# francescofugazzi/3dgsconverter

Hardware: NVIDIA H100
Metric: Msplats/s SOR k=16 (higher is better)
Workload: dtype f32

## Files before the change

3dgsconverter_b200/csrc/gsx_radix.cu:

```cuda
#include "../../include/gsx.h"

#include "gsx_common.cuh"
#include "gsx_radix.cuh"

namespace gsx {

#define GSX_FULL 0xffffffffu
constexpr int kRsThreads = 256;
constexpr int kRsPerThread = 16;
constexpr int kRsTile = kRsThreads * kRsPerThread;
constexpr int kRsWarpKeys = 32 * kRsPerThread;
constexpr int kScanBlock = 2048;

__global__ void __launch_bounds__(256) k_scan_block(uint32_t* __restrict__ data, int64_t n,
                                                    uint32_t* __restrict__ sums) {
    const int64_t base = (int64_t)blockIdx.x * kScanBlock + (int64_t)threadIdx.x * 8;
    uint32_t v[8];
    uint32_t tsum = 0;
#pragma unroll
    for (int e = 0; e < 8; ++e) {
        v[e] = base + e < n ? data[base + e] : 0u;
        tsum += v[e];
    }
    uint32_t x = tsum;
// ... 114 lines not shown
    __syncthreads();
    uint32_t dcount;
    {
        const int d = threadIdx.x;
        uint32_t run = 0;
#pragma unroll
        for (int ww = 0; ww < 8; ++ww) {
            uint32_t c = wcnt[ww][d];
            wcnt[ww][d] = run;
            run += c;
        }
        dcount = run;
        gbase[d] = base_off[(size_t)d * ntiles + blockIdx.x];
    }
    {
        uint32_t x = dcount;
#pragma unroll
        for (int o = 1; o < 32; o <<= 1) {
            uint32_t y = __shfl_up_sync(GSX_FULL, x, o);
            if (lane >= o) x += y;
        }
        __shared__ uint32_t wtot[8];
        if (lane == 31) wtot[w] = x;
        __syncthreads();
        uint32_t woff = 0;
#pragma unroll
        for (int i = 0; i < 8; ++i)
            if (i < w) woff += wtot[i];
        dstart[threadIdx.x] = woff + x - dcount;
    }
    __syncthreads();
#pragma unroll
    for (int e = 0; e < kRsPerThread; ++e) {
        const int64_t i = wbase + e * 32 + lane;
        if (i < n) {
            const uint32_t d = (uint32_t)(key[e] >> shift) & dmask;
            const uint32_t lp = dstart[d] + wcnt[w][d] + rank[e];
            skeys[lp] = key[e];
            svals[lp] = vals_in[i];
        }
    }
    __syncthreads();
    const int cnt = (int)(n - tbase < kRsTile ? n - tbase : kRsTile);
    for (int j = threadIdx.x; j < cnt; j += kRsThreads) {
        const uint64_t k = skeys[j];
        const uint32_t d = (uint32_t)(k >> shift) & dmask;
        const uint32_t pos = gbase[d] + ((uint32_t)j - dstart[d]);
        keys_out[pos] = k;
        vals_out[pos] = svals[j];
    }
}

constexpr uint32_t kOsAgg = 1u << 30, kOsInc = 1u << 31, kOsVal = (1u << 30) - 1u;
constexpr int kOsMaxPass = 8;
constexpr uint32_t kOsSpinLimit = 1u << 22;

__global__ void __launch_bounds__(256) k_os_hist(const uint64_t* __restrict__ keys, int64_t n, int begin_bit,
                                                  int npass, uint32_t last_mask, uint32_t* __restrict__ ghist) {
    __shared__ uint32_t sh[kOsMaxPass * 256];
    for (int t = threadIdx.x; t < npass * 256; t += 256) sh[t] = 0;
    __syncthreads();
    const int64_t stride = (int64_t)gridDim.x * 256;
    for (int64_t i = (int64_t)blockIdx.x * 256 + threadIdx.x; i < n; i += stride) {
        const uint64_t k = keys[i] >> begin_bit;
        for (int p = 0; p < npass; ++p)
            atomicAdd(&sh[p * 256 + ((uint32_t)(k >> (8 * p)) & (p == npass - 1 ? last_mask : 255u))], 1u);
    }
    __syncthreads();
    for (int t = threadIdx.x; t < npass * 256; t += 256)
        if (sh[t]) atomicAdd(&ghist[t], sh[t]);
}

__global__ void __launch_bounds__(256) k_os_scan(uint32_t* __restrict__ ghist) {
    uint32_t* h = ghist + blockIdx.x * 256;
    const int lane = threadIdx.x & 31, w = threadIdx.x >> 5;
    const uint32_t v = h[threadIdx.x];
    uint32_t x = v;
#pragma unroll
    for (int o = 1; o < 32; o <<= 1) {
        uint32_t y = __shfl_up_sync(GSX_FULL, x, o);
        if (lane >= o) x += y;
    }
    __shared__ uint32_t wt[8];
    if (lane == 31) wt[w] = x;
    __syncthreads();
    uint32_t woff = 0;
#pragma unroll
    for (int i = 0; i < 8; ++i)
        if (i < w) woff += wt[i];
    h[threadIdx.x] = woff + x - v;
}

template <bool PAIRS>
constexpr size_t os_pass_smem() {
    return (size_t)kRsTile * (PAIRS ? 12 : 8) + (size_t)8 * 256 * 4 + 2 * 256 * 4;
}

template <bool PAIRS>
__global__ void __launch_bounds__(kRsThreads, PAIRS ? 3 : 4)
    k_os_pass(const uint64_t* __restrict__ keys_in, const int32_t* __restrict__ vals_in, uint64_t* __restrict__ keys_out,
              int32_t* __restrict__ vals_out, int64_t n, int shift, uint32_t dmask, const uint32_t* __restrict__ gbase_pass,
              uint32_t* lookback, unsigned int* tile_counter) {
    extern __shared__ __align__(16) unsigned char rs_smem[];
    uint64_t* skeys = reinterpret_cast<uint64_t*>(rs_smem);
    int32_t* svals = reinterpret_cast<int32_t*>(rs_smem + (size_t)kRsTile * 8);
    constexpr size_t kPairBytes = (size_t)kRsTile * (PAIRS ? 12 : 8);
    uint32_t(*wcnt)[256] = reinterpret_cast<uint32_t(*)[256]>(rs_smem + kPairBytes);
    uint32_t* dstart = reinterpret_cast<uint32_t*>(rs_smem + kPairBytes + 8 * 256 * 4);
    uint32_t* gbase = dstart + 256;
    __shared__ unsigned int s_tile;
    const int lane = threadIdx.x & 31, w = threadIdx.x >> 5;
    if (threadIdx.x == 0) s_tile = atomicAdd(tile_counter, 1u);
    for (int t = threadIdx.x; t < 8 * 256; t += kRsThreads) (&wcnt[0][0])[t] = 0;
    __syncthreads();
    const unsigned int tile = s_tile;
    const int64_t tbase = (int64_t)tile * kRsTile;
    const int64_t wbase = tbase + (int64_t)w * kRsWarpKeys;
    uint64_t key[kRsPerThread];
    uint32_t rank2[kRsPerThread / 2];
#pragma unroll
    for (int e = 0; e < kRsPerThread; ++e) {
        const int64_t i = wbase + e * 32 + lane;
        key[e] = i < n ? keys_in[i] : 0ull;
// ... 30 lines not shown
        for (int64_t t = (int64_t)tile - 1; t >= 0; --t) {
            uint32_t v, spins = 0;
            while (((v = lb[(size_t)t * 256 + d]) & (kOsAgg | kOsInc)) == 0u)
                if (++spins > kOsSpinLimit) __trap();
            excl += v & kOsVal;
            if (v & kOsInc) break;
        }
        if (tile != 0) lb[(size_t)tile * 256 + d] = (excl + dcount) | kOsInc;
        gbase[d] = gbase_pass[d] + excl;
    }
    {
        uint32_t x = dcount;
#pragma unroll
        for (int o = 1; o < 32; o <<= 1) {
            uint32_t y = __shfl_up_sync(GSX_FULL, x, o);
            if (lane >= o) x += y;
        }
        __shared__ uint32_t wtot[8];
        if (lane == 31) wtot[w] = x;
        __syncthreads();
        uint32_t woff = 0;
#pragma unroll
        for (int i = 0; i < 8; ++i)
            if (i < w) woff += wtot[i];
        dstart[threadIdx.x] = woff + x - dcount;
    }
    __syncthreads();
#pragma unroll
    for (int e = 0; e < kRsPerThread; ++e) {
        const int64_t i = wbase + e * 32 + lane;
        if (i < n) {
            const uint32_t d = (uint32_t)(key[e] >> shift) & dmask;
            const uint32_t lp = dstart[d] + wcnt[w][d] + ((rank2[e >> 1] >> (16 * (e & 1))) & 0xffffu);
            skeys[lp] = key[e];
            if (PAIRS) svals[lp] = vals_in[i];
        }
    }
    __syncthreads();
    const int cnt = (int)(n - tbase < kRsTile ? n - tbase : kRsTile);
    for (int j = threadIdx.x; j < cnt; j += kRsThreads) {
        const uint64_t k = skeys[j];
        const uint32_t d = (uint32_t)(k >> shift) & dmask;
        const uint32_t pos = gbase[d] + ((uint32_t)j - dstart[d]);
        keys_out[pos] = k;
        if (PAIRS) vals_out[pos] = svals[j];
    }
}

static size_t os_ws_elems(int64_t n) {
    const int64_t ntiles = (n + kRsTile - 1) / kRsTile;
    return (size_t)kOsMaxPass * 256 + 64 + (size_t)kOsMaxPass * 256 * ntiles;
}

template <bool PAIRS>
static int onesweep_sort(uint64_t* keys0, uint64_t* keys1, int32_t* vals0, int32_t* vals1, int64_t n, int begin_bit,
                         int end_bit, uint32_t* ws, uint64_t** keys_sorted, int32_t** vals_sorted, cudaStream_t st) {
    const int64_t ntiles = (n + kRsTile - 1) / kRsTile;
    const int npass = (end_bit - begin_bit + 7) / 8;
    uint32_t* ghist = ws;
    unsigned int* counters = ws + kOsMaxPass * 256;
    uint32_t* lookback = ws + kOsMaxPass * 256 + 64;
    GSX_CUDA_CHECK(cudaMemsetAsync(ws, 0, ((size_t)kOsMaxPass * 256 + 64 + (size_t)npass * 256 * ntiles) * sizeof(uint32_t), st));
    static int hist_blocks = 0;
    if (!hist_blocks) {
        int dev = 0, sms = 132;
        cudaGetDevice(&dev);
        cudaDeviceGetAttribute(&sms, cudaDevAttrMultiProcessorCount, dev);
        hist_blocks = sms * 8;
    }
    int64_t hb = (n + 255) / 256;
    if (hb > hist_blocks) hb = hist_blocks;
    const uint32_t last_mask = digit_mask(begin_bit + 8 * (npass - 1), end_bit);
    k_os_hist<<<(unsigned)hb, 256, 0, st>>>(keys0, n, begin_bit, npass, last_mask, ghist);
    GSX_KERNEL_CHECK();
    k_os_scan<<<npass, 256, 0, st>>>(ghist);
    GSX_KERNEL_CHECK();
    GSX_CUDA_CHECK(cudaFuncSetAttribute(k_os_pass<PAIRS>, cudaFuncAttributeMaxDynamicSharedMemorySize, (int)os_pass_smem<PAIRS>()));
    uint64_t *kin = keys0, *kout = keys1;
    int32_t *vin = vals0, *vout = vals1;
    for (int p = 0; p < npass; ++p) {
        k_os_pass<PAIRS><<<(unsigned)ntiles, kRsThreads, os_pass_smem<PAIRS>(), st>>>(
            kin, vin, kout, vout, n, begin_bit + 8 * p, p == npass - 1 ? last_mask : 255u, ghist + p * 256,
            lookback + (size_t)p * 256 * ntiles, counters + p);
        GSX_KERNEL_CHECK();
        uint64_t* tk = kin;
        kin = kout;
        kout = tk;
        int32_t* tv = vin;
        vin = vout;
        vout = tv;
    }
    *keys_sorted = kin;
    if (vals_sorted) *vals_sorted = vin;
    return GSX_OK;
}

size_t radix_ws_bytes(int64_t n) {
    if (n < 1) n = 1;
    int64_t ntiles = (n + kRsTile - 1) / kRsTile;
    size_t hist = (size_t)256 * ntiles;
    size_t three_kernel = hist + scan_ws_elems((int64_t)hist) + 256;
    size_t onesweep = os_ws_elems(n);
    return (three_kernel > onesweep ? three_kernel : onesweep) * sizeof(uint32_t);
}

int radix_sort_pairs(uint64_t* keys0, uint64_t* keys1, int32_t* vals0, int32_t* vals1, int64_t n, int begin_bit,
                     int end_bit, void* ws, size_t ws_bytes, uint64_t** keys_sorted, int32_t** vals_sorted,
                     cudaStream_t st) {
    GSX_NVTX("gsx::radix_sort_pairs");
    GSX_REQUIRE(n >= 1 && n < 4294967296ll, GSX_ERR_ARG, "radix: n out of range");
    GSX_REQUIRE(ws_bytes >= radix_ws_bytes(n), GSX_ERR_WORKSPACE, "radix: workspace too small");
    GSX_REQUIRE(begin_bit >= 0 && end_bit <= 64 && begin_bit < end_bit, GSX_ERR_ARG, "radix: bad bit range");
    if (n < (1ll << 30))
        return onesweep_sort<true>(keys0, keys1, vals0, vals1, n, begin_bit, end_bit, (uint32_t*)ws, keys_sorted,
                                   vals_sorted, st);
    const int64_t ntiles = (n + kRsTile - 1) / kRsTile;
    uint32_t* hist = (uint32_t*)ws;
    uint32_t* scan_ws = hist + (size_t)256 * ntiles;
    GSX_CUDA_CHECK(cudaFuncSetAttribute(k_rs_scatter, cudaFuncAttributeMaxDynamicSharedMemorySize, (int)kRsScatterSmem));
    uint64_t *kin = keys0, *kout = keys1;
    int32_t *vin = vals0, *vout = vals1;
    for (int shift = begin_bit; shift < end_bit; shift += 8) {
        const uint32_t dmask = digit_mask(shift, end_bit);
        k_rs_hist<<<(unsigned)ntiles, kRsThreads, 0, st>>>(kin, n, shift, dmask, ntiles, hist);
        GSX_KERNEL_CHECK();
        int rc = exclusive_scan_u32(hist, (int64_t)256 * ntiles, scan_ws, st);
        if (rc) return rc;
        k_rs_scatter<<<(unsigned)ntiles, kRsThreads, kRsScatterSmem, st>>>(kin, vin, kout, vout, n, shift, dmask, ntiles,
                                                                          hist);
        GSX_KERNEL_CHECK();
        uint64_t* tk = kin;
        kin = kout;
        kout = tk;
        int32_t* tv = vin;
        vin = vout;
        vout = tv;
    }
    *keys_sorted = kin;
    *vals_sorted = vin;
    return GSX_OK;
}

int radix_sort_keys(uint64_t* keys0, uint64_t* keys1, int64_t n, int begin_bit, int end_bit, void* ws, size_t ws_bytes,
                    uint64_t** keys_sorted, cudaStream_t st) {
    GSX_NVTX("gsx::radix_sort_keys");
    GSX_REQUIRE(n >= 1 && n < (1ll << 30), GSX_ERR_ARG, "radix: n out of range");
    GSX_REQUIRE(ws_bytes >= radix_ws_bytes(n), GSX_ERR_WORKSPACE, "radix: workspace too small");
    GSX_REQUIRE(begin_bit >= 0 && end_bit <= 64 && begin_bit < end_bit, GSX_ERR_ARG, "radix: bad bit range");
    return onesweep_sort<false>(keys0, keys1, nullptr, nullptr, n, begin_bit, end_bit, (uint32_t*)ws, keys_sorted, nullptr,
                                st);
}

}

using namespace gsx;

extern "C" {

int64_t gsx_sort_pairs_workspace_bytes(int64_t n) {
    if (n < 1) n = 1;
    return (int64_t)(align_up((size_t)n * 8, 256) + align_up((size_t)n * 4, 256) + radix_ws_bytes(n) + 1024);
}

int gsx_sort_pairs(uint64_t* keys_dev, int32_t* vals_dev, int64_t n, int32_t begin_bit, int32_t end_bit, void* ws,
                   int64_t ws_bytes, void* stream) {
    cudaStream_t st = (cudaStream_t)stream;
    if (n == 0) return GSX_OK;
    GSX_REQUIRE(ws_bytes >= gsx_sort_pairs_workspace_bytes(n), GSX_ERR_WORKSPACE, "sort: workspace too small");
    Carver c(ws, (size_t)ws_bytes);
    uint64_t* k1 = c.take<uint64_t>((size_t)n);
    int32_t* v1 = c.take<int32_t>((size_t)n);
    char* rws = c.take<char>(radix_ws_bytes(n));
    uint64_t* ks = nullptr;
    int32_t* vs = nullptr;
    int rc = vals_dev ? radix_sort_pairs(keys_dev, k1, vals_dev, v1, n, begin_bit, end_bit, rws, radix_ws_bytes(n), &ks,
                                         &vs, st)
                      : radix_sort_keys(keys_dev, k1, n, begin_bit, end_bit, rws, radix_ws_bytes(n), &ks, st);
    if (rc) return rc;
    if (ks != keys_dev) {
        GSX_CUDA_CHECK(cudaMemcpyAsync(keys_dev, ks, (size_t)n * 8, cudaMemcpyDeviceToDevice, st));
        if (vals_dev) GSX_CUDA_CHECK(cudaMemcpyAsync(vals_dev, vs, (size_t)n * 4, cudaMemcpyDeviceToDevice, st));
    }
    return GSX_OK;
}

}
```

3dgsconverter_b200/csrc/gsx_radix.cuh:

```cuda
#pragma once
#include "gsx_common.cuh"
namespace gsx {
size_t radix_ws_bytes(int64_t n);
size_t scan_workspace_bytes(int64_t n);
int exclusive_scan_u32_ws(uint32_t* data, int64_t n, uint32_t* ws, cudaStream_t st);
int radix_sort_pairs(uint64_t* keys0, uint64_t* keys1, int32_t* vals0, int32_t* vals1, int64_t n, int begin_bit,
                     int end_bit, void* ws, size_t ws_bytes, uint64_t** keys_sorted, int32_t** vals_sorted,
                     cudaStream_t st);
int radix_sort_keys(uint64_t* keys0, uint64_t* keys1, int64_t n, int begin_bit, int end_bit, void* ws, size_t ws_bytes,
                    uint64_t** keys_sorted, cudaStream_t st);
}
```

3dgsconverter_b200/csrc/gsx_sor.cu:

```cuda
#include "../../include/gsx.h"

#include "gsx_common.cuh"
#include "gsx_sor.cuh"

#include "gsx_radix.cuh"
#include <math.h>

namespace gsx {

#define GSX_D2LIM_BITS 0x60ad78ebu
#define GSX_FULL 0xffffffffu

constexpr int kCellCodeBits = 15;
constexpr float kCellCodeScale = (float)(1 << (kCellCodeBits / 3));
constexpr float kCellCodeMax = kCellCodeScale - 1.f;
constexpr int kSmallBucket = 64;
constexpr int kQueryBatch = 16;
constexpr int kMergeThreshold = 9;
constexpr int kKnnMinBlocks = 8;
constexpr int kFlatSupers = 8;
const char* sor_build_info() {
    return "knn=r03a;epi_smem=1;first_sort=1;query_batch=16;minblocks=8;merge_threshold=9;small_bucket=64;"
           "flat_supers=8;knn16=0;tma=0;i32=1;cell_order=hilbert15";
}
// ... 140 lines not shown
    }
    y ^= x, z ^= y;
    uint32_t t = 0;
#pragma unroll
    for (uint32_t q = 16; q > 1; q >>= 1)
        if (z & q) t ^= q - 1;
    x ^= t, y ^= t, z ^= t;
    return (spread6(x) << 2) | (spread6(y) << 1) | spread6(z);
}

__device__ __forceinline__ uint64_t bucket_key(float x, float y, float z, float bx, float by, float bz, float cell,
                                               int64_t n, uint64_t M64) {
    float fx, fy, fz, flx, fly, flz;
    const uint32_t h = bucket_hash(x, y, z, bx, by, bz, cell, n, M64, fx, fy, fz, flx, fly, flz);
    uint32_t sx = (uint32_t)fminf(kCellCodeMax, fmaxf(0.f, (fx - flx) * kCellCodeScale));
    uint32_t sy = (uint32_t)fminf(kCellCodeMax, fmaxf(0.f, (fy - fly) * kCellCodeScale));
    uint32_t sz = (uint32_t)fminf(kCellCodeMax, fmaxf(0.f, (fz - flz) * kCellCodeScale));
    return ((uint64_t)h << kCellCodeBits) | (uint64_t)hilbert15(sx, sy, sz);
}

struct PackFmt {
    int idx_bits, mort_bits, bucket_bits;
    __host__ __device__ int key_shift() const { return idx_bits + mort_bits; }
    __host__ __device__ uint64_t idx_mask() const { return (1ull << idx_bits) - 1ull; }
    __host__ __device__ int sort_begin() const { return idx_bits; }
    __host__ __device__ int sort_end() const { return idx_bits + mort_bits + bucket_bits; }
};

static int bits_for(int64_t n) {
    int b = 1;
    while (((int64_t)1 << b) < n) ++b;
    return b;
}

static PackFmt pack_fmt(int64_t n_items, int64_t n_buckets) {
    PackFmt f;
    f.idx_bits = bits_for(n_items);
    f.bucket_bits = bits_for(n_buckets);
    int avail = 64 - f.idx_bits - f.bucket_bits;
    if (avail > kCellCodeBits) avail = kCellCodeBits;
    f.mort_bits = avail < 0 ? 0 : avail - avail % 3;
    return f;
}

__device__ __forceinline__ uint64_t pack_word(uint64_t key , uint64_t bucket_sub,
                                              int64_t idx, PackFmt f) {
    const uint64_t bucket = (key >> kCellCodeBits) - bucket_sub;
    const uint64_t mort = (key & ((1ull << kCellCodeBits) - 1ull)) >> (kCellCodeBits - f.mort_bits);
    return (((bucket << f.mort_bits) | mort) << f.idx_bits) | (uint64_t)idx;
}

__global__ void __launch_bounds__(256) k_sor_keys(const float* __restrict__ xyz, int64_t n, float bx, float by,
                                                  float bz, float cell, uint64_t M64, PackFmt f,
                                                  uint64_t* __restrict__ keys) {
    int64_t i = (int64_t)blockIdx.x * blockDim.x + threadIdx.x;
    if (i >= n) return;
    keys[i] = pack_word(bucket_key(xyz[3 * i], xyz[3 * i + 1], xyz[3 * i + 2], bx, by, bz, cell, n, M64), 0, i, f);
}

__device__ __forceinline__ uint32_t float_to_ord(float f) {
    const uint32_t u = __float_as_uint(f);
    return (u & 0x80000000u) ? ~u : (u | 0x80000000u);
}
__device__ __forceinline__ float ord_to_float(uint32_t o) {
    return __uint_as_float((o & 0x80000000u) ? (o & 0x7fffffffu) : ~o);
}

template <bool GATHER>
__device__ __forceinline__ void
    sor_finish_tile(const int64_t tile, const float* __restrict__ xyz, const uint64_t* __restrict__ keys, PackFmt fmt,
                    float4* __restrict__ spos, int64_t n, float bx, float by, float bz, float cell, uint64_t M64,
                    int2* __restrict__ tab_se, uint32_t* __restrict__ startbits, uint32_t* __restrict__ cellbits,
                    float4* __restrict__ caabb, float4* __restrict__ saabb) {
    const int64_t j = tile * 1024 + threadIdx.x;
    const int lane = lane_id();
    float lo[3] = {INFINITY, INFINITY, INFINITY}, hi[3] = {-INFINITY, -INFINITY, -INFINITY};
    uint32_t h = 0xffffffffu;
    auto hash_at = [&](int64_t t) -> uint32_t {
        if (GATHER) return (uint32_t)(keys[t] >> fmt.key_shift());
        const float4 q = spos[t];
        return bucket_of(q.x, q.y, q.z, bx, by, bz, cell, n, M64);
    };
    int gcx = 0x7fffffff, gcy = 0, gcz = 0;
    if (j < n) {
        float x, y, z;
        if (GATHER) {
            const uint64_t word = keys[j];
            const int32_t idx = (int32_t)(word & fmt.idx_mask());
            x = xyz[3 * (int64_t)idx], y = xyz[3 * (int64_t)idx + 1], z = xyz[3 * (int64_t)idx + 2];
            spos[j] = make_float4(x, y, z, __int_as_float(idx));
            h = (uint32_t)(word >> fmt.key_shift());
        } else {
            const float4 p = spos[j];
            x = p.x, y = p.y, z = p.z;
            h = bucket_of(x, y, z, bx, by, bz, cell, n, M64);
        }
        gcx = (int)floorf(__fdiv_rn(__fsub_rn(x, bx), cell));
        gcy = (int)floorf(__fdiv_rn(__fsub_rn(y, by), cell));
        gcz = (int)floorf(__fdiv_rn(__fsub_rn(z, bz), cell));
        lo[0] = hi[0] = x;
        lo[1] = hi[1] = y;
        lo[2] = hi[2] = z;
    }
    __shared__ uint32_t sh_h[1024];
    sh_h[threadIdx.x] = h;
    __syncthreads();
    uint32_t hprev = threadIdx.x > 0 ? sh_h[threadIdx.x - 1] : 0xffffffffu;
    uint32_t hnext = threadIdx.x < 1023 ? sh_h[threadIdx.x + 1] : 0xffffffffu;
    if (j < n) {
        if (threadIdx.x == 0 && j > 0) hprev = hash_at(j - 1);
// ... 50 lines not shown
}

template <bool GATHER>
__global__ void __launch_bounds__(1024)
    k_sor_finish(const float* __restrict__ xyz, const uint64_t* __restrict__ keys, PackFmt fmt,
                 float4* __restrict__ spos, int64_t n, float bx, float by, float bz, float cell, uint64_t M64,
                 int2* __restrict__ tab_se, uint32_t* __restrict__ startbits, uint32_t* __restrict__ cellbits,
                 float4* __restrict__ caabb, float4* __restrict__ saabb) {
    sor_finish_tile<GATHER>(blockIdx.x, xyz, keys, fmt, spos, n, bx, by, bz, cell, M64, tab_se, startbits, cellbits, caabb,
                            saabb);
}

__global__ void __launch_bounds__(1024)
    k_sor_finish_gated(float4* __restrict__ spos, int64_t n, float bx, float by, float bz, float cell, uint64_t M64,
                       int2* __restrict__ tab_se, uint32_t* __restrict__ startbits, uint32_t* __restrict__ cellbits,
                       float4* __restrict__ caabb, float4* __restrict__ saabb, const unsigned int* __restrict__ gate) {
    if (!*gate) return;
    const int64_t tiles = (n + 1023) / 1024;
    for (int64_t t = blockIdx.x; t < tiles; t += gridDim.x) {
        sor_finish_tile<false>(t, nullptr, nullptr, PackFmt{}, spos, n, bx, by, bz, cell, M64, tab_se, startbits, cellbits,
                               caabb, saabb);
        __syncthreads();
    }
}

__device__ __forceinline__ void bucket_box_partial(const float4* __restrict__ spos, const float4* __restrict__ caabb,
                                                   int64_t s, int64_t end, int lane, float (&lo)[3], float (&hi)[3]) {
    lo[0] = lo[1] = lo[2] = INFINITY;
    hi[0] = hi[1] = hi[2] = -INFINITY;
    int64_t cf = (s + 31) >> 5, cl = end >> 5;
    int64_t head_end = cf * 32, tail_begin = cl * 32;
    if (cf > cl) {
        head_end = end;
        tail_begin = end;
        cf = cl = 0;
    }
    for (int64_t t = s + lane; t < head_end; t += 32) {
        float4 p = spos[t];
        lo[0] = fminf(lo[0], p.x), lo[1] = fminf(lo[1], p.y), lo[2] = fminf(lo[2], p.z);
        hi[0] = fmaxf(hi[0], p.x), hi[1] = fmaxf(hi[1], p.y), hi[2] = fmaxf(hi[2], p.z);
    }
    for (int64_t c = cf + lane; c < cl; c += 32) {
        float4 a = caabb[2 * c], b = caabb[2 * c + 1];
        lo[0] = fminf(lo[0], a.x), lo[1] = fminf(lo[1], a.y), lo[2] = fminf(lo[2], a.z);
        hi[0] = fmaxf(hi[0], a.w), hi[1] = fmaxf(hi[1], b.x), hi[2] = fmaxf(hi[2], b.y);
    }
    for (int64_t t = tail_begin + lane; t < end; t += 32) {
        float4 p = spos[t];
        lo[0] = fminf(lo[0], p.x), lo[1] = fminf(lo[1], p.y), lo[2] = fminf(lo[2], p.z);
        hi[0] = fmaxf(hi[0], p.x), hi[1] = fmaxf(hi[1], p.y), hi[2] = fmaxf(hi[2], p.z);
    }
}

__device__ __forceinline__ void
    bucket_boxes_chunk(const int64_t chunk, const uint32_t* __restrict__ startbits, const float4* __restrict__ spos,
                       const float4* __restrict__ caabb, const int2* __restrict__ tab_se, int64_t n, float bx,
                       float by, float bz, float cell, uint64_t M64, float4* __restrict__ tab_box) {
    const int lane = lane_id();
    if (chunk * 32 >= n) return;
    unsigned m = startbits[chunk];
    uint32_t my_h = 0;
    int my_end = 0;
    if ((m >> lane) & 1u) {
        const float4 p0 = spos[chunk * 32 + lane];
        my_h = bucket_of(p0.x, p0.y, p0.z, bx, by, bz, cell, n, M64);
        my_end = tab_se[my_h].y;
    }
    while (m) {
        const int src = __ffs(m) - 1;
        m &= m - 1;
        const int64_t s = chunk * 32 + src;
        const uint32_t hb = __shfl_sync(GSX_FULL, my_h, src);
        const int64_t end = __shfl_sync(GSX_FULL, my_end, src);
        float lo[3], hi[3];
        bucket_box_partial(spos, caabb, s, end, lane, lo, hi);
#pragma unroll
        for (int a = 0; a < 3; ++a)
#pragma unroll
            for (int o = 16; o > 0; o >>= 1) {
                lo[a] = fminf(lo[a], __shfl_xor_sync(GSX_FULL, lo[a], o));
                hi[a] = fmaxf(hi[a], __shfl_xor_sync(GSX_FULL, hi[a], o));
            }
        if (lane == 0) {
            tab_box[2 * (size_t)hb] = make_float4(lo[0], lo[1], lo[2], 0.f);
            tab_box[2 * (size_t)hb + 1] = make_float4(hi[0], hi[1], hi[2], 0.f);
        }
    }
}

__global__ void __launch_bounds__(256)
    k_sor_bucket_boxes(const uint32_t* __restrict__ startbits, const float4* __restrict__ spos,
                       const float4* __restrict__ caabb, const int2* __restrict__ tab_se, int64_t n, float bx,
                       float by, float bz, float cell, uint64_t M64, float4* __restrict__ tab_box) {
    bucket_boxes_chunk(((int64_t)blockIdx.x * blockDim.x + threadIdx.x) >> 5, startbits, spos, caabb, tab_se, n, bx, by, bz,
                       cell, M64, tab_box);
}

__global__ void __launch_bounds__(256)
    k_sor_bucket_boxes_gated(const uint32_t* __restrict__ startbits, const float4* __restrict__ spos,
                             const float4* __restrict__ caabb, const int2* __restrict__ tab_se, int64_t n, float bx,
                             float by, float bz, float cell, uint64_t M64, float4* __restrict__ tab_box,
                             const unsigned int* __restrict__ gate) {
    if (!*gate) return;
    const int64_t nchunk = (n + 31) >> 5, step = ((int64_t)gridDim.x * blockDim.x) >> 5;
    for (int64_t c = ((int64_t)blockIdx.x * blockDim.x + threadIdx.x) >> 5; c < nchunk; c += step)
        bucket_boxes_chunk(c, startbits, spos, caabb, tab_se, n, bx, by, bz, cell, M64, tab_box);
}

struct StartList {
    unsigned int* count;
    unsigned int* pos;
    unsigned int capacity;
};

__global__ void __launch_bounds__(1024)
    k_sor_finish_flags(const float4* __restrict__ spos, const uint8_t* __restrict__ flags, int64_t n,
                       uint32_t* __restrict__ startbits, uint32_t* __restrict__ cellbits, float4* __restrict__ caabb,
                       float4* __restrict__ saabb, StartList sl) {
    const int64_t j = (int64_t)blockIdx.x * 1024 + threadIdx.x;
    const int lane = lane_id();
    float lo[3] = {INFINITY, INFINITY, INFINITY}, hi[3] = {-INFINITY, -INFINITY, -INFINITY};
    bool start = false, newcell = false;
    if (j < n) {
        const float4 p = spos[j];
        lo[0] = hi[0] = p.x;
        lo[1] = hi[1] = p.y;
        lo[2] = hi[2] = p.z;
        const uint8_t f = flags[j];
        start = (f & 1) != 0;
        newcell = (f & 2) != 0;
    }
    const unsigned sb = __ballot_sync(GSX_FULL, start), cb = __ballot_sync(GSX_FULL, newcell);
    __shared__ unsigned s_wcnt[32], s_base;
    const int w = threadIdx.x >> 5;
    if (lane == 0) s_wcnt[w] = __popc(sb);
#pragma unroll
    for (int a = 0; a < 3; ++a) {
        lo[a] = ord_to_float(__reduce_min_sync(GSX_FULL, float_to_ord(lo[a])));
        hi[a] = ord_to_float(__reduce_max_sync(GSX_FULL, float_to_ord(hi[a])));
    }
    __shared__ float sm[6][32];
    const int64_t chunk = (int64_t)blockIdx.x * 32 + w;
    if (lane == 0) {
        if (chunk * 32 < n) {
            startbits[chunk] = sb;
            cellbits[chunk] = cb;
            caabb[2 * chunk] = make_float4(lo[0], lo[1], lo[2], hi[0]);
            caabb[2 * chunk + 1] = make_float4(hi[1], hi[2], 0.f, 0.f);
        }
        for (int a = 0; a < 3; ++a) {
            sm[a][w] = lo[a];
            sm[3 + a][w] = hi[a];
        }
    }
    __syncthreads();
    if (w == 0) {
        unsigned v = s_wcnt[lane], x = v;
#pragma unroll
        for (int o = 1; o < 32; o <<= 1) {
// ... 33 lines not shown
}

__global__ void __launch_bounds__(256)
    k_sor_bucket_tail(const float4* __restrict__ spos, const uint8_t* __restrict__ flags, int64_t n, float bx, float by,
                      float bz, float cell, uint64_t M64, int2* __restrict__ tab_se, float4* __restrict__ tab_box,
                      uint32_t* __restrict__ bigbits, StartList sl) {
    if (sl.count[1]) return;
    const unsigned t = blockIdx.x * blockDim.x + threadIdx.x;
    if (t >= sl.count[0]) return;
    const int64_t pj = sl.pos[t];
    const float4 p = spos[pj];
    const uint32_t h = bucket_of(p.x, p.y, p.z, bx, by, bz, cell, n, M64);
    float blo[3] = {p.x, p.y, p.z}, bhi[3] = {p.x, p.y, p.z};
    int64_t u = pj + 1;
    const int64_t lim = pj + kSmallBucket < n ? pj + kSmallBucket : n;
    for (; u < lim; ++u) {
        if (flags[u] & 1) break;
        const float4 c = spos[u];
        blo[0] = fminf(blo[0], c.x), blo[1] = fminf(blo[1], c.y), blo[2] = fminf(blo[2], c.z);
        bhi[0] = fmaxf(bhi[0], c.x), bhi[1] = fmaxf(bhi[1], c.y), bhi[2] = fmaxf(bhi[2], c.z);
    }
    const bool closed = u == n || (flags[u] & 1);
    if (closed) {
        tab_se[h] = make_int2((int)pj, (int)u);
        tab_box[2 * (size_t)h] = make_float4(blo[0], blo[1], blo[2], 0.f);
        tab_box[2 * (size_t)h + 1] = make_float4(bhi[0], bhi[1], bhi[2], 0.f);
    } else {
        tab_se[h].x = (int)pj;
        atomicOr(bigbits + (pj >> 5), 1u << (pj & 31));
    }
}

__global__ void __launch_bounds__(256)
    k_sor_big_buckets(const uint32_t* __restrict__ bigbits, const uint32_t* __restrict__ startbits,
                      const float4* __restrict__ spos, const float4* __restrict__ caabb, int64_t n, float bx, float by,
                      float bz, float cell, uint64_t M64, int2* __restrict__ tab_se, float4* __restrict__ tab_box,
                      StartList sl) {
    if (sl.count[1]) return;
    const int lane = lane_id();
    const int64_t nchunk = (n + 31) >> 5;
    const int64_t wstep = (((int64_t)gridDim.x * blockDim.x) >> 5) * 32;
    for (int64_t c0 = (((int64_t)blockIdx.x * blockDim.x + threadIdx.x) >> 5) * 32; c0 < nchunk; c0 += wstep) {
    const uint32_t myword = c0 + lane < nchunk ? bigbits[c0 + lane] : 0u;
    unsigned wordmask = __ballot_sync(GSX_FULL, myword != 0u);
    while (wordmask) {
    const int wl = __ffs(wordmask) - 1;
    wordmask &= wordmask - 1;
    const int64_t chunk = c0 + wl;
    unsigned m = __shfl_sync(GSX_FULL, myword, wl);
    while (m) {
        const int src = __ffs(m) - 1;
        m &= m - 1;
        const int64_t s = chunk * 32 + src;
        int64_t end = n;
        {
            const unsigned rest = src == 31 ? 0u : (startbits[chunk] & (0xffffffffu << (src + 1)));
            if (rest) {
                end = chunk * 32 + __ffs(rest) - 1;
            } else {
                for (int64_t d0 = chunk + 1; d0 < nchunk; d0 += 32) {
                    const int64_t c = d0 + lane;
                    const unsigned wv = c < nchunk ? startbits[c] : 0u;
                    const unsigned any = __ballot_sync(GSX_FULL, wv != 0u);
                    if (any) {
                        const int l = __ffs(any) - 1;
                        const unsigned word = __shfl_sync(GSX_FULL, wv, l);
                        end = (d0 + l) * 32 + __ffs(word) - 1;
                        break;
                    }
                }
            }
        }
        const float4 p0 = spos[s];
        const uint32_t hb = bucket_of(p0.x, p0.y, p0.z, bx, by, bz, cell, n, M64);
        float lo[3], hi[3];
        bucket_box_partial(spos, caabb, s, end, lane, lo, hi);
#pragma unroll
        for (int a = 0; a < 3; ++a) {
            lo[a] = ord_to_float(__reduce_min_sync(GSX_FULL, float_to_ord(lo[a])));
            hi[a] = ord_to_float(__reduce_max_sync(GSX_FULL, float_to_ord(hi[a])));
        }
        if (lane == 0) {
            tab_se[hb].y = (int)end;
            tab_box[2 * (size_t)hb] = make_float4(lo[0], lo[1], lo[2], 0.f);
            tab_box[2 * (size_t)hb + 1] = make_float4(hi[0], hi[1], hi[2], 0.f);
        }
    }
    }
    }
}

template <bool GATHER>
static int sor_finish(const float* xyz, int64_t n, const float* bmin, float cell, SorWs& w, PackFmt fmt, cudaStream_t st) {
    const uint64_t M64 = 0xFFFFFFFFFFFFFFFFull / (uint64_t)n;
    GSX_CUDA_CHECK(cudaMemsetAsync(w.tab_se, 0, (size_t)n * sizeof(int2), st));
    k_sor_finish<GATHER><<<(int)((n + 1023) / 1024), 1024, 0, st>>>(xyz, w.keys_sorted, fmt, w.spos, n, bmin[0],
                                                                    bmin[1], bmin[2], cell, M64, w.tab_se, w.startbits,
                                                                    w.cellbits, w.caabb, w.saabb);
    GSX_KERNEL_CHECK();
    k_sor_bucket_boxes<<<(int)((n + 255) / 256), 256, 0, st>>>(w.startbits, w.spos, w.caabb, w.tab_se, n, bmin[0],
                                                               bmin[1], bmin[2], cell, M64, w.tab_box);
    GSX_KERNEL_CHECK();
    return GSX_OK;
}

int sor_build(const float* xyz, int64_t n, const float* bmin, float cell, SorWs& w, cudaStream_t st) {
    GSX_NVTX("gsx::sor_build");
    int blocks = (int)((n + 255) / 256);
    const PackFmt fmt = pack_fmt(n, n);
    k_sor_keys<<<blocks, 256, 0, st>>>(xyz, n, bmin[0], bmin[1], bmin[2], cell, 0xFFFFFFFFFFFFFFFFull / (uint64_t)n,
                                       fmt, w.keys0);
    GSX_KERNEL_CHECK();
    {
        int rc = radix_sort_keys(w.keys0, w.keys1, n, fmt.sort_begin(), fmt.sort_end(), w.sort_ws, w.sort_ws_bytes,
                                 &w.keys_sorted, st);
        if (rc) return rc;
    }
    return sor_finish<true>(xyz, n, bmin, cell, w, fmt, st);
}


__global__ void __launch_bounds__(256) k_sor_owner_keys(const float* __restrict__ xyz, int64_t n, int64_t n_global,
                                                        int world, float bx, float by, float bz, float cell,
                                                        uint64_t M64, int idx_bits, uint64_t* __restrict__ keys) {
    int64_t i = (int64_t)blockIdx.x * blockDim.x + threadIdx.x;
    if (i >= n) return;
    uint64_t h = bucket_key(xyz[3 * i], xyz[3 * i + 1], xyz[3 * i + 2], bx, by, bz, cell, n_global, M64) >> kCellCodeBits;
    keys[i] = (((h * (uint64_t)world) / (uint64_t)n_global) << idx_bits) | (uint64_t)i;
}

__global__ void __launch_bounds__(256) k_sor_gather_slab(const float* __restrict__ xyz,
                                                         const uint64_t* __restrict__ words, uint64_t idx_mask, int64_t n,
                                                         int64_t idx_base, float4* __restrict__ pos4) {
    int64_t j = (int64_t)blockIdx.x * blockDim.x + threadIdx.x;
    if (j >= n) return;
    int32_t idx = (int32_t)(words[j] & idx_mask);
    pos4[j] = make_float4(xyz[3 * (int64_t)idx], xyz[3 * (int64_t)idx + 1], xyz[3 * (int64_t)idx + 2],
                          __int_as_float((int)(idx_base + idx)));
}

__global__ void k_sor_owner_counts(const uint64_t* __restrict__ owners_sorted, int idx_bits, int64_t n, int world,
                                   long long* __restrict__ cuts) {
    int o = threadIdx.x;
    if (o > world) return;
    int64_t lo = 0, hi = n;
    while (lo < hi) {
        int64_t mid = (lo + hi) >> 1;
        if ((owners_sorted[mid] >> idx_bits) < (uint64_t)o) lo = mid + 1; else hi = mid;
    }
    cuts[o] = lo;
}

int sor_dist_local_run(const float* xyz, int64_t n_local, int64_t idx_base, int64_t n_global, int world,
                       const float* bmin, float cell, float4* pos4_out, long long* cuts_dev, SorWs& w,
                       cudaStream_t st) {
    GSX_NVTX("gsx::sor_dist_local_run");
    GSX_REQUIRE(world >= 1 && world <= 255, GSX_ERR_ARG, "sor: world size must be in [1,255]");
    if (n_local == 0) {
        GSX_CUDA_CHECK(cudaMemsetAsync(cuts_dev, 0, (size_t)(world + 1) * sizeof(long long), st));
        return GSX_OK;
    }
    int blocks = (int)((n_local + 255) / 256);
    const int idx_bits = bits_for(n_local);
    k_sor_owner_keys<<<blocks, 256, 0, st>>>(xyz, n_local, n_global, world, bmin[0], bmin[1], bmin[2], cell,
                                             0xFFFFFFFFFFFFFFFFull / (uint64_t)n_global, idx_bits, w.keys0);
    GSX_KERNEL_CHECK();
    uint64_t* ks = nullptr;
    int rc = radix_sort_keys(w.keys0, w.keys1, n_local, idx_bits, idx_bits + 8, w.sort_ws, w.sort_ws_bytes, &ks,
                             st);
    if (rc) return rc;
// ... 44 lines not shown

int sor_dist_merge(const float4* pos4_in, int64_t m, int64_t n_global, int64_t bucket_lo, int64_t bucket_hi,
                   const float* bmin, float cell, float4* pos4_out, uint8_t* flags_out, SorWs& w, cudaStream_t st) {
    GSX_NVTX("gsx::sor_dist_merge");
    if (m == 0) return GSX_OK;
    GSX_REQUIRE(bucket_lo >= 0 && bucket_lo < bucket_hi && bucket_hi <= n_global, GSX_ERR_ARG, "sor: bad bucket range");
    int blocks = (int)((m + 255) / 256);
    const PackFmt fmt = pack_fmt(m, bucket_hi - bucket_lo);
    k_sor_keys_pos4<<<blocks, 256, 0, st>>>(pos4_in, m, n_global, bmin[0], bmin[1], bmin[2], cell,
                                            0xFFFFFFFFFFFFFFFFull / (uint64_t)n_global, (uint64_t)bucket_lo, fmt, w.keys0);
    GSX_KERNEL_CHECK();
    uint64_t* ks = nullptr;
    int rc = radix_sort_keys(w.keys0, w.keys1, m, fmt.sort_begin(), fmt.sort_end(), w.sort_ws, w.sort_ws_bytes, &ks, st);
    if (rc) return rc;
    if (flags_out)
        k_owner_gather_flags<<<blocks, 256, 0, st>>>(pos4_in, ks, fmt, m, bmin[0], bmin[1], bmin[2], cell, pos4_out,
                                                     flags_out);
    else
        k_gather4<<<blocks, 256, 0, st>>>(pos4_in, ks, fmt.idx_mask(), m, pos4_out);
    GSX_KERNEL_CHECK();
    return GSX_OK;
}

int sor_build_from_sorted(const float4* spos_in, const uint8_t* flags, int64_t n, const float* bmin, float cell, SorWs& w,
                          cudaStream_t st) {
    GSX_NVTX("gsx::sor_build_from_sorted");
    if (spos_in != w.spos)
        GSX_CUDA_CHECK(cudaMemcpyAsync(w.spos, spos_in, (size_t)n * sizeof(float4), cudaMemcpyDeviceToDevice, st));
    w.keys_sorted = nullptr;
    if (!flags) return sor_finish<false>(nullptr, n, bmin, cell, w, PackFmt{}, st);
    const uint64_t M64 = 0xFFFFFFFFFFFFFFFFull / (uint64_t)n;
    const int64_t nchunk = (n + 31) / 32;
    StartList sl;
    sl.count = w.counters + 8;
    sl.pos = reinterpret_cast<unsigned int*>(w.startlist);
    sl.capacity = (unsigned)(n / 8 + 1024);
    GSX_CUDA_CHECK(cudaMemsetAsync(w.tab_se, 0, (size_t)n * sizeof(int2), st));
    GSX_CUDA_CHECK(cudaMemsetAsync(w.bigbits, 0, (size_t)nchunk * sizeof(uint32_t), st));
    GSX_CUDA_CHECK(cudaMemsetAsync(sl.count, 0, 2 * sizeof(unsigned int), st));
    k_sor_finish_flags<<<(int)((n + 1023) / 1024), 1024, 0, st>>>(w.spos, flags, n, w.startbits, w.cellbits, w.caabb,
                                                                  w.saabb, sl);
    GSX_KERNEL_CHECK();
    const unsigned tail_blocks = (sl.capacity + 255) / 256;
    k_sor_bucket_tail<<<tail_blocks, 256, 0, st>>>(w.spos, flags, n, bmin[0], bmin[1], bmin[2], cell, M64, w.tab_se,
                                                   w.tab_box, w.bigbits, sl);
    GSX_KERNEL_CHECK();
    k_sor_big_buckets<<<sm_count() * 8, 256, 0, st>>>(w.bigbits, w.startbits, w.spos, w.caabb, n, bmin[0], bmin[1], bmin[2],
                                                      cell, M64, w.tab_se, w.tab_box, sl);
    GSX_KERNEL_CHECK();
    const int resident = sm_count() * 2;
    k_sor_finish_gated<<<resident, 1024, 0, st>>>(w.spos, n, bmin[0], bmin[1], bmin[2], cell, M64, w.tab_se, w.startbits,
                                                  w.cellbits, w.caabb, w.saabb, sl.count + 1);
    GSX_KERNEL_CHECK();
    k_sor_bucket_boxes_gated<<<resident * 4, 256, 0, st>>>(w.startbits, w.spos, w.caabb, w.tab_se, n, bmin[0], bmin[1],
                                                           bmin[2], cell, M64, w.tab_box, sl.count + 1);
    GSX_KERNEL_CHECK();
    return GSX_OK;
}


__device__ __forceinline__ uint32_t probe_hash(int nx, int ny, int nz, uint32_t n, uint64_t M, int mode) {
    if (mode == GSX_HASH_MODE_I32WRAP) {
        int32_t h = (int32_t)((uint32_t)nx * 73856093u) ^ (int32_t)((uint32_t)ny * 19349663u) ^
                    (int32_t)((uint32_t)nz * 83492791u);
        uint32_t a = h < 0 ? (uint32_t)(-(int64_t)h) : (uint32_t)h;
        uint32_t r = fastmod_u32(a, M, n);
        return h < 0 ? (r ? n - r : 0u) : r;
    } else {
        int64_t h = ((int64_t)nx * 73856093LL) ^ ((int64_t)ny * 19349663LL) ^ ((int64_t)nz * 83492791LL);
        int64_t r = h % (int64_t)n;
        if (r < 0) r += n;
        return (uint32_t)r;
    }
}

constexpr unsigned kKeyNone = 0xffffffffu;
__device__ __forceinline__ unsigned knn_key(float lb, int lane) { return (__float_as_uint(lb) & ~31u) | (unsigned)lane; }
__device__ __forceinline__ float knn_key_lb(unsigned key) { return __uint_as_float(key & ~31u); }

__device__ __forceinline__ float box_lb(const float4* __restrict__ aabb, int64_t id, float qx, float qy, float qz) {
    float4 a = __ldg(aabb + 2 * id), b = __ldg(aabb + 2 * id + 1);
    float dx = fmaxf(fmaxf(__fsub_rn(a.x, qx), __fsub_rn(qx, a.w)), 0.f);
    float dy = fmaxf(fmaxf(__fsub_rn(a.y, qy), __fsub_rn(qy, b.x)), 0.f);
    float dz = fmaxf(fmaxf(__fsub_rn(a.z, qz), __fsub_rn(qz, b.y)), 0.f);
    return __fadd_rn(__fadd_rn(__fmul_rn(dx, dx), __fmul_rn(dy, dy)), __fmul_rn(dz, dz));
}

__device__ __forceinline__ float cmpx(float v, int j, bool take_min) {
    float o = __shfl_xor_sync(GSX_FULL, v, j);
    return take_min ? fminf(v, o) : fmaxf(v, o);
}

__device__ __forceinline__ float warp_sort32(float v, int lane) {
#pragma unroll
    for (int k = 2; k <= 32; k <<= 1) {
#pragma unroll
        for (int j = k >> 1; j > 0; j >>= 1) v = cmpx(v, j, ((lane & k) == 0) == ((lane & j) == 0));
    }
    return v;
}

template <int NREG>
struct TopK {
    float v0, v1;
    float tau;
    int K;
    __device__ __forceinline__ void init(int k) {
        K = k;
// ... 494 lines not shown
```

Baseline: 1286.

## Fuse onesweep histogram into SOR key generation and derive bucket ends from startbits

The SOR key-generation kernel now also builds the onesweep radix histogram in shared memory while writing keys, so the separate histogram kernel and its re-read of the key array are skipped through a new 'counted' flag. The kernel becomes grid-stride with a capped block count. Bucket box construction no longer reads tab_se for bucket ends. It finds them by scanning startbits, and in the gather path it takes the bucket hash from the sorted key instead of recomputing it from positions. The trade-offs are extra shared-memory atomics in the key kernel and possible warp-wide startbits scans for long buckets.

```diff
diff --git a/3dgsconverter_b200/csrc/gsx_radix.cu b/3dgsconverter_b200/csrc/gsx_radix.cu
--- a/3dgsconverter_b200/csrc/gsx_radix.cu
+++ b/3dgsconverter_b200/csrc/gsx_radix.cu
@@ -190,23 +190,16 @@
 }
 
 constexpr uint32_t kOsAgg = 1u << 30, kOsInc = 1u << 31, kOsVal = (1u << 30) - 1u;
-constexpr int kOsMaxPass = 8;
 constexpr uint32_t kOsSpinLimit = 1u << 22;
 
-__global__ void __launch_bounds__(256) k_os_hist(const uint64_t* __restrict__ keys, int64_t n, int begin_bit,
-                                                  int npass, uint32_t last_mask, uint32_t* __restrict__ ghist) {
+__global__ void __launch_bounds__(256) k_os_hist(const uint64_t* __restrict__ keys, int64_t n, OsHist hist) {
     __shared__ uint32_t sh[kOsMaxPass * 256];
-    for (int t = threadIdx.x; t < npass * 256; t += 256) sh[t] = 0;
+    for (int t = threadIdx.x; t < hist.npass * 256; t += 256) sh[t] = 0;
     __syncthreads();
     const int64_t stride = (int64_t)gridDim.x * 256;
-    for (int64_t i = (int64_t)blockIdx.x * 256 + threadIdx.x; i < n; i += stride) {
-        const uint64_t k = keys[i] >> begin_bit;
-        for (int p = 0; p < npass; ++p)
-            atomicAdd(&sh[p * 256 + ((uint32_t)(k >> (8 * p)) & (p == npass - 1 ? last_mask : 255u))], 1u);
-    }
-    __syncthreads();
-    for (int t = threadIdx.x; t < npass * 256; t += 256)
-        if (sh[t]) atomicAdd(&ghist[t], sh[t]);
+    for (int64_t i = (int64_t)blockIdx.x * 256 + threadIdx.x; i < n; i += stride) os_hist_add(sh, keys[i], hist);
+    __syncthreads();
+    os_hist_flush(sh, hist);
 }
 
 __global__ void __launch_bounds__(256) k_os_scan(uint32_t* __restrict__ ghist) {
@@ -343,27 +336,36 @@
     return (size_t)kOsMaxPass * 256 + 64 + (size_t)kOsMaxPass * 256 * ntiles;
 }
 
+static int os_prepare(int64_t n, int begin_bit, int end_bit, uint32_t* ws, OsHist* hist, cudaStream_t st) {
+    const int64_t ntiles = (n + kRsTile - 1) / kRsTile;
+    const int npass = (end_bit - begin_bit + 7) / 8;
+    GSX_CUDA_CHECK(cudaMemsetAsync(ws, 0, ((size_t)kOsMaxPass * 256 + 64 + (size_t)npass * 256 * ntiles) * sizeof(uint32_t), st));
+    *hist = OsHist{ws, begin_bit, npass, digit_mask(begin_bit + 8 * (npass - 1), end_bit)};
+    return GSX_OK;
+}
+
+int64_t os_hist_blocks(int64_t n) {
+    const int64_t b = (n + 255) / 256, cap = (int64_t)sm_count() * 8;
+    return b < cap ? b : cap;
+}
+
 template <bool PAIRS>
 static int onesweep_sort(uint64_t* keys0, uint64_t* keys1, int32_t* vals0, int32_t* vals1, int64_t n, int begin_bit,
-                         int end_bit, uint32_t* ws, uint64_t** keys_sorted, int32_t** vals_sorted, cudaStream_t st) {
+                         int end_bit, uint32_t* ws, uint64_t** keys_sorted, int32_t** vals_sorted, cudaStream_t st,
+                         bool counted) {
     const int64_t ntiles = (n + kRsTile - 1) / kRsTile;
     const int npass = (end_bit - begin_bit + 7) / 8;
+    const uint32_t last_mask = digit_mask(begin_bit + 8 * (npass - 1), end_bit);
     uint32_t* ghist = ws;
     unsigned int* counters = ws + kOsMaxPass * 256;
     uint32_t* lookback = ws + kOsMaxPass * 256 + 64;
-    GSX_CUDA_CHECK(cudaMemsetAsync(ws, 0, ((size_t)kOsMaxPass * 256 + 64 + (size_t)npass * 256 * ntiles) * sizeof(uint32_t), st));
-    static int hist_blocks = 0;
-    if (!hist_blocks) {
-        int dev = 0, sms = 132;
-        cudaGetDevice(&dev);
-        cudaDeviceGetAttribute(&sms, cudaDevAttrMultiProcessorCount, dev);
-        hist_blocks = sms * 8;
-    }
-    int64_t hb = (n + 255) / 256;
-    if (hb > hist_blocks) hb = hist_blocks;
-    const uint32_t last_mask = digit_mask(begin_bit + 8 * (npass - 1), end_bit);
-    k_os_hist<<<(unsigned)hb, 256, 0, st>>>(keys0, n, begin_bit, npass, last_mask, ghist);
-    GSX_KERNEL_CHECK();
+    if (!counted) {
+        OsHist hist;
+        const int rc = os_prepare(n, begin_bit, end_bit, ws, &hist, st);
+        if (rc) return rc;
+        k_os_hist<<<(unsigned)os_hist_blocks(n), 256, 0, st>>>(keys0, n, hist);
+        GSX_KERNEL_CHECK();
+    }
     k_os_scan<<<npass, 256, 0, st>>>(ghist);
     GSX_KERNEL_CHECK();
     GSX_CUDA_CHECK(cudaFuncSetAttribute(k_os_pass<PAIRS>, cudaFuncAttributeMaxDynamicSharedMemorySize, (int)os_pass_smem<PAIRS>()));
@@ -404,7 +406,7 @@
     GSX_REQUIRE(begin_bit >= 0 && end_bit <= 64 && begin_bit < end_bit, GSX_ERR_ARG, "radix: bad bit range");
     if (n < (1ll << 30))
         return onesweep_sort<true>(keys0, keys1, vals0, vals1, n, begin_bit, end_bit, (uint32_t*)ws, keys_sorted,
-                                   vals_sorted, st);
+                                   vals_sorted, st, false);
     const int64_t ntiles = (n + kRsTile - 1) / kRsTile;
     uint32_t* hist = (uint32_t*)ws;
     uint32_t* scan_ws = hist + (size_t)256 * ntiles;
@@ -432,14 +434,22 @@
     return GSX_OK;
 }
 
+#define GSX_RADIX_KEYS_REQUIRE()                                                                                    \
+    GSX_REQUIRE(n >= 1 && n < (1ll << 30), GSX_ERR_ARG, "radix: n out of range");                                   \
+    GSX_REQUIRE(ws_bytes >= radix_ws_bytes(n), GSX_ERR_WORKSPACE, "radix: workspace too small");                    \
+    GSX_REQUIRE(begin_bit >= 0 && end_bit <= 64 && begin_bit < end_bit, GSX_ERR_ARG, "radix: bad bit range")
+
+int radix_keys_prepare(int64_t n, int begin_bit, int end_bit, void* ws, size_t ws_bytes, OsHist* hist, cudaStream_t st) {
+    GSX_RADIX_KEYS_REQUIRE();
+    return os_prepare(n, begin_bit, end_bit, (uint32_t*)ws, hist, st);
+}
+
 int radix_sort_keys(uint64_t* keys0, uint64_t* keys1, int64_t n, int begin_bit, int end_bit, void* ws, size_t ws_bytes,
-                    uint64_t** keys_sorted, cudaStream_t st) {
+                    uint64_t** keys_sorted, cudaStream_t st, bool counted) {
     GSX_NVTX("gsx::radix_sort_keys");
-    GSX_REQUIRE(n >= 1 && n < (1ll << 30), GSX_ERR_ARG, "radix: n out of range");
-    GSX_REQUIRE(ws_bytes >= radix_ws_bytes(n), GSX_ERR_WORKSPACE, "radix: workspace too small");
-    GSX_REQUIRE(begin_bit >= 0 && end_bit <= 64 && begin_bit < end_bit, GSX_ERR_ARG, "radix: bad bit range");
+    GSX_RADIX_KEYS_REQUIRE();
     return onesweep_sort<false>(keys0, keys1, nullptr, nullptr, n, begin_bit, end_bit, (uint32_t*)ws, keys_sorted, nullptr,
-                                st);
+                                st, counted);
 }
 
 }
diff --git a/3dgsconverter_b200/csrc/gsx_radix.cuh b/3dgsconverter_b200/csrc/gsx_radix.cuh
--- a/3dgsconverter_b200/csrc/gsx_radix.cuh
+++ b/3dgsconverter_b200/csrc/gsx_radix.cuh
@@ -7,6 +7,25 @@
 int radix_sort_pairs(uint64_t* keys0, uint64_t* keys1, int32_t* vals0, int32_t* vals1, int64_t n, int begin_bit,
                      int end_bit, void* ws, size_t ws_bytes, uint64_t** keys_sorted, int32_t** vals_sorted,
                      cudaStream_t st);
+
+constexpr int kOsMaxPass = 8;
+struct OsHist {
+    uint32_t* ghist;
+    int begin_bit, npass;
+    uint32_t last_mask;
+};
+__device__ __forceinline__ void os_hist_add(uint32_t* sh , uint64_t key, const OsHist& h) {
+    const uint64_t k = key >> h.begin_bit;
+    for (int p = 0; p < h.npass; ++p)
+        atomicAdd(&sh[p * 256 + ((uint32_t)(k >> (8 * p)) & (p == h.npass - 1 ? h.last_mask : 255u))], 1u);
+}
+__device__ __forceinline__ void os_hist_flush(const uint32_t* sh, const OsHist& h) {
+    for (int t = threadIdx.x; t < h.npass * 256; t += blockDim.x)
+        if (sh[t]) atomicAdd(&h.ghist[t], sh[t]);
+}
+int64_t os_hist_blocks(int64_t n);
+int radix_keys_prepare(int64_t n, int begin_bit, int end_bit, void* ws, size_t ws_bytes, OsHist* hist, cudaStream_t st);
+
 int radix_sort_keys(uint64_t* keys0, uint64_t* keys1, int64_t n, int begin_bit, int end_bit, void* ws, size_t ws_bytes,
-                    uint64_t** keys_sorted, cudaStream_t st);
+                    uint64_t** keys_sorted, cudaStream_t st, bool counted = false);
 }
diff --git a/3dgsconverter_b200/csrc/gsx_sor.cu b/3dgsconverter_b200/csrc/gsx_sor.cu
--- a/3dgsconverter_b200/csrc/gsx_sor.cu
+++ b/3dgsconverter_b200/csrc/gsx_sor.cu
@@ -216,10 +216,19 @@
 
 __global__ void __launch_bounds__(256) k_sor_keys(const float* __restrict__ xyz, int64_t n, float bx, float by,
                                                   float bz, float cell, uint64_t M64, PackFmt f,
-                                                  uint64_t* __restrict__ keys) {
-    int64_t i = (int64_t)blockIdx.x * blockDim.x + threadIdx.x;
-    if (i >= n) return;
-    keys[i] = pack_word(bucket_key(xyz[3 * i], xyz[3 * i + 1], xyz[3 * i + 2], bx, by, bz, cell, n, M64), 0, i, f);
+                                                  uint64_t* __restrict__ keys, OsHist hist) {
+    __shared__ uint32_t sh[kOsMaxPass * 256];
+    for (int t = threadIdx.x; t < hist.npass * 256; t += 256) sh[t] = 0;
+    __syncthreads();
+    const int64_t stride = (int64_t)gridDim.x * 256;
+    for (int64_t i = (int64_t)blockIdx.x * 256 + threadIdx.x; i < n; i += stride) {
+        const uint64_t word =
+            pack_word(bucket_key(xyz[3 * i], xyz[3 * i + 1], xyz[3 * i + 2], bx, by, bz, cell, n, M64), 0, i, f);
+        keys[i] = word;
+        os_hist_add(sh, word, hist);
+    }
+    __syncthreads();
+    os_hist_flush(sh, hist);
 }
 
 __device__ __forceinline__ uint32_t float_to_ord(float f) {
@@ -376,26 +385,46 @@
     }
 }
 
+__device__ __forceinline__ int64_t bucket_end(const uint32_t* __restrict__ startbits, unsigned word, int64_t chunk,
+                                              int src, int64_t n, int lane) {
+    const unsigned rest = src == 31 ? 0u : (word & (0xffffffffu << (src + 1)));
+    if (rest) return chunk * 32 + __ffs(rest) - 1;
+    const int64_t nchunk = (n + 31) >> 5;
+    for (int64_t d0 = chunk + 1; d0 < nchunk; d0 += 32) {
+        const int64_t c = d0 + lane;
+        const unsigned wv = c < nchunk ? startbits[c] : 0u;
+        const unsigned any = __ballot_sync(GSX_FULL, wv != 0u);
+        if (any) {
+            const int l = __ffs(any) - 1;
+            return (d0 + l) * 32 + __ffs(__shfl_sync(GSX_FULL, wv, l)) - 1;
+        }
+    }
+    return n;
+}
+
+template <bool GATHER>
 __device__ __forceinline__ void
-    bucket_boxes_chunk(const int64_t chunk, const uint32_t* __restrict__ startbits, const float4* __restrict__ spos,
-                       const float4* __restrict__ caabb, const int2* __restrict__ tab_se, int64_t n, float bx,
-                       float by, float bz, float cell, uint64_t M64, float4* __restrict__ tab_box) {
+    bucket_boxes_chunk(const int64_t chunk, const unsigned word, const uint32_t* __restrict__ startbits,
+                       const float4* __restrict__ spos,
+                       const float4* __restrict__ caabb, const uint64_t* __restrict__ keys, PackFmt fmt, int64_t n,
+                       float bx, float by, float bz, float cell, uint64_t M64, float4* __restrict__ tab_box) {
     const int lane = lane_id();
-    if (chunk * 32 >= n) return;
-    unsigned m = startbits[chunk];
     uint32_t my_h = 0;
-    int my_end = 0;
-    if ((m >> lane) & 1u) {
-        const float4 p0 = spos[chunk * 32 + lane];
-        my_h = bucket_of(p0.x, p0.y, p0.z, bx, by, bz, cell, n, M64);
-        my_end = tab_se[my_h].y;
-    }
+    if ((word >> lane) & 1u) {
+        if (GATHER) {
+            my_h = (uint32_t)(keys[chunk * 32 + lane] >> fmt.key_shift());
+        } else {
+            const float4 p0 = spos[chunk * 32 + lane];
+            my_h = bucket_of(p0.x, p0.y, p0.z, bx, by, bz, cell, n, M64);
+        }
+    }
+    unsigned m = word;
     while (m) {
         const int src = __ffs(m) - 1;
         m &= m - 1;
         const int64_t s = chunk * 32 + src;
         const uint32_t hb = __shfl_sync(GSX_FULL, my_h, src);
-        const int64_t end = __shfl_sync(GSX_FULL, my_end, src);
+        const int64_t end = bucket_end(startbits, word, chunk, src, n, lane);
         float lo[3], hi[3];
         bucket_box_partial(spos, caabb, s, end, lane, lo, hi);
 #pragma unroll
@@ -412,23 +441,26 @@
     }
 }
 
+template <bool GATHER>
 __global__ void __launch_bounds__(256)
     k_sor_bucket_boxes(const uint32_t* __restrict__ startbits, const float4* __restrict__ spos,
-                       const float4* __restrict__ caabb, const int2* __restrict__ tab_se, int64_t n, float bx,
-                       float by, float bz, float cell, uint64_t M64, float4* __restrict__ tab_box) {
-    bucket_boxes_chunk(((int64_t)blockIdx.x * blockDim.x + threadIdx.x) >> 5, startbits, spos, caabb, tab_se, n, bx, by, bz,
-                       cell, M64, tab_box);
+                       const float4* __restrict__ caabb, const uint64_t* __restrict__ keys, PackFmt fmt, int64_t n,
+                       float bx, float by, float bz, float cell, uint64_t M64, float4* __restrict__ tab_box) {
+    const int64_t chunk = ((int64_t)blockIdx.x * blockDim.x + threadIdx.x) >> 5;
+    if (chunk * 32 >= n) return;
+    bucket_boxes_chunk<GATHER>(chunk, startbits[chunk], startbits, spos, caabb, keys, fmt, n, bx, by, bz, cell, M64,
+                               tab_box);
 }
 
 __global__ void __launch_bounds__(256)
     k_sor_bucket_boxes_gated(const uint32_t* __restrict__ startbits, const float4* __restrict__ spos,
-                             const float4* __restrict__ caabb, const int2* __restrict__ tab_se, int64_t n, float bx,
-                             float by, float bz, float cell, uint64_t M64, float4* __restrict__ tab_box,
-                             const unsigned int* __restrict__ gate) {
+                             const float4* __restrict__ caabb, int64_t n, float bx, float by, float bz, float cell,
+                             uint64_t M64, float4* __restrict__ tab_box, const unsigned int* __restrict__ gate) {
     if (!*gate) return;
     const int64_t nchunk = (n + 31) >> 5, step = ((int64_t)gridDim.x * blockDim.x) >> 5;
     for (int64_t c = ((int64_t)blockIdx.x * blockDim.x + threadIdx.x) >> 5; c < nchunk; c += step)
-        bucket_boxes_chunk(c, startbits, spos, caabb, tab_se, n, bx, by, bz, cell, M64, tab_box);
+        bucket_boxes_chunk<false>(c, startbits[c], startbits, spos, caabb, nullptr, PackFmt{}, n, bx, by, bz, cell, M64,
+                                  tab_box);
 }
 
 struct StartList {
@@ -568,25 +600,7 @@
         const int src = __ffs(m) - 1;
         m &= m - 1;
         const int64_t s = chunk * 32 + src;
-        int64_t end = n;
-        {
-            const unsigned rest = src == 31 ? 0u : (startbits[chunk] & (0xffffffffu << (src + 1)));
-            if (rest) {
-                end = chunk * 32 + __ffs(rest) - 1;
-            } else {
-                for (int64_t d0 = chunk + 1; d0 < nchunk; d0 += 32) {
-                    const int64_t c = d0 + lane;
-                    const unsigned wv = c < nchunk ? startbits[c] : 0u;
-                    const unsigned any = __ballot_sync(GSX_FULL, wv != 0u);
-                    if (any) {
-                        const int l = __ffs(any) - 1;
-                        const unsigned word = __shfl_sync(GSX_FULL, wv, l);
-                        end = (d0 + l) * 32 + __ffs(word) - 1;
-                        break;
-                    }
-                }
-            }
-        }
+        const int64_t end = bucket_end(startbits, startbits[chunk], chunk, src, n, lane);
         const float4 p0 = spos[s];
         const uint32_t hb = bucket_of(p0.x, p0.y, p0.z, bx, by, bz, cell, n, M64);
         float lo[3], hi[3];
@@ -614,24 +628,24 @@
                                                                     bmin[1], bmin[2], cell, M64, w.tab_se, w.startbits,
                                                                     w.cellbits, w.caabb, w.saabb);
     GSX_KERNEL_CHECK();
-    k_sor_bucket_boxes<<<(int)((n + 255) / 256), 256, 0, st>>>(w.startbits, w.spos, w.caabb, w.tab_se, n, bmin[0],
-                                                               bmin[1], bmin[2], cell, M64, w.tab_box);
+    k_sor_bucket_boxes<GATHER><<<(int)((n + 255) / 256), 256, 0, st>>>(w.startbits, w.spos, w.caabb, w.keys_sorted, fmt,
+                                                                       n, bmin[0], bmin[1], bmin[2], cell, M64, w.tab_box);
     GSX_KERNEL_CHECK();
     return GSX_OK;
 }
 
 int sor_build(const float* xyz, int64_t n, const float* bmin, float cell, SorWs& w, cudaStream_t st) {
     GSX_NVTX("gsx::sor_build");
-    int blocks = (int)((n + 255) / 256);
     const PackFmt fmt = pack_fmt(n, n);
-    k_sor_keys<<<blocks, 256, 0, st>>>(xyz, n, bmin[0], bmin[1], bmin[2], cell, 0xFFFFFFFFFFFFFFFFull / (uint64_t)n,
-                                       fmt, w.keys0);
-    GSX_KERNEL_CHECK();
-    {
-        int rc = radix_sort_keys(w.keys0, w.keys1, n, fmt.sort_begin(), fmt.sort_end(), w.sort_ws, w.sort_ws_bytes,
-                                 &w.keys_sorted, st);
-        if (rc) return rc;
-    }
+    OsHist hist;
+    int rc = radix_keys_prepare(n, fmt.sort_begin(), fmt.sort_end(), w.sort_ws, w.sort_ws_bytes, &hist, st);
+    if (rc) return rc;
+    k_sor_keys<<<(unsigned)os_hist_blocks(n), 256, 0, st>>>(xyz, n, bmin[0], bmin[1], bmin[2], cell,
+                                                            0xFFFFFFFFFFFFFFFFull / (uint64_t)n, fmt, w.keys0, hist);
+    GSX_KERNEL_CHECK();
+    rc = radix_sort_keys(w.keys0, w.keys1, n, fmt.sort_begin(), fmt.sort_end(), w.sort_ws, w.sort_ws_bytes,
+                         &w.keys_sorted, st, true);
+    if (rc) return rc;
     return sor_finish<true>(xyz, n, bmin, cell, w, fmt, st);
 }
 
@@ -782,8 +796,8 @@
     k_sor_finish_gated<<<resident, 1024, 0, st>>>(w.spos, n, bmin[0], bmin[1], bmin[2], cell, M64, w.tab_se, w.startbits,
                                                   w.cellbits, w.caabb, w.saabb, sl.count + 1);
     GSX_KERNEL_CHECK();
-    k_sor_bucket_boxes_gated<<<resident * 4, 256, 0, st>>>(w.startbits, w.spos, w.caabb, w.tab_se, n, bmin[0], bmin[1],
-                                                           bmin[2], cell, M64, w.tab_box, sl.count + 1);
+    k_sor_bucket_boxes_gated<<<resident * 4, 256, 0, st>>>(w.startbits, w.spos, w.caabb, n, bmin[0], bmin[1], bmin[2],
+                                                           cell, M64, w.tab_box, sl.count + 1);
     GSX_KERNEL_CHECK();
     return GSX_OK;
 }
```

New measurement: 1290, median of 6. Within noise of the previous version (+0.3%).
